# CornellHPC/HySortK

Hardware: AMD Instinct MI355X
Metric: k-mers counted/sec at K=31 (higher is better)
Workload: dtype u64

## Files before the change

hysortk_amd/csrc/hsk_api.hip:

```cpp
#include <hip/hip_runtime.h>
#include <dlfcn.h>
#include <algorithm>
#include <cstdarg>
#include <cstdio>
#include <cstdlib>
#include <cstring>
#include <future>
#include <map>
#include <string>
#include <thread>
#include <type_traits>
#include <vector>

#include "../../include/hsk.h"
#include "hsk_device.h"
#include "hsk_parse.h"
#include "hsk_expand.h"
#include "hsk_sort.h"
#include "hsk_scatter.h"
#include "hsk_count.h"
#include "hsk_finish.h"
#include "hsk_agg.h"
#include "hsk_combine.h"
#include "hsk_heavy.h"
#include "hsk_pairs.h"
#include "hsk_pairmerge.h"
#include "hsk_pairdiag.h"
#include "hsk_strand.h"
#include "hsk_estimate.h"
#include "hsk_synth.h"
#include "hsk_plan.h"
#include "hsk_tuning.h"
#include "hsk_comm.h"

using namespace hsk;

#include "hsk_pool.h"
#include "hsk_host_ctx.h"

extern "C" int hsk_abi_version(void) { return HSK_ABI_VERSION; }

extern "C" void *hsk_host_alloc(uint64_t bytes)
{
    void *p = nullptr;
    if (hipHostMalloc(&p, bytes ? bytes : 64, hipHostMallocDefault) != hipSuccess) { (void)hipGetLastError(); return nullptr; }
    return p;
}
extern "C" void hsk_host_free(void *p) { if (p) (void)hipHostFree(p); }

extern "C" int hsk_device_count(void)
{
    int n = 0;
    if (hipGetDeviceCount(&n) != hipSuccess) { (void)hipGetLastError(); return 0; }
    return n;
}

extern "C" const char *hsk_strerror(int s)
{
    switch (s) {
    case HSK_OK: return "ok";
    case HSK_ERR_INVALID_ARG: return "invalid argument";
    case HSK_ERR_NO_DEVICE: return "no usable HIP device (gfx950 required; there is no CPU fallback)";
    case HSK_ERR_HIP: return "HIP runtime error";
    case HSK_ERR_OOM: return "out of memory";
    case HSK_ERR_DISPATCH: return "Cannot dispatch tasks. May be too unbalanced.";
    case HSK_ERR_INTERNAL: return "internal device-side check failed";
    case HSK_ERR_COMM: return "RCCL communication error";
    case HSK_ERR_UNSUPPORTED: return "not supported";
    default: return "unknown status";
    }
}

extern "C" const char *hsk_last_error(const hsk_ctx *c) { return c ? c->err : ""; }

extern "C" void hsk_config_default(hsk_config *cfg)
{
    memset(cfg, 0, sizeof *cfg);
    cfg->kmer_size = 31; cfg->minimizer_size = 17; cfg->lower_freq = 15; cfg->upper_freq = 40;
    cfg->extension = 0; cfg->ntasks = 0; cfg->device = 0; cfg->plain_dispatcher = 0;
    cfg->dispatch_upper_coe = 1.5; cfg->dispatch_step = 0.05; cfg->radix_bits = 8; cfg->flags = 0; cfg->unbalanced_ratio = 2.3;
}

static int validate_cfg(const hsk_config *cfg)
{
    const int K = cfg->kmer_size, M = cfg->minimizer_size;
    if (!(2 < K && K < 96) || (K % 32) == 0) return 0;
    if (!(0 < M && M < K) || (M % 32) == 0) return 0;
    if (!(0 < cfg->lower_freq && cfg->lower_freq <= cfg->upper_freq && cfg->upper_freq <= 65535)) return 0;
    if (cfg->extension != 0 && cfg->extension != 1) return 0;
    if (cfg->ntasks < 0 || cfg->ntasks > HSK_MAX_TASKS) return 0;
    if (cfg->radix_bits != 0 && (cfg->radix_bits < MIN_RADIX_BITS || cfg->radix_bits > MAX_RADIX_BITS)) return 0;
    return 1;
}

#include <execinfo.h>
#include <signal.h>
#include <unistd.h>
static void backtrace_on_abort(int sig)
{
    void *frames[64];
    const int n = backtrace(frames, 64);
    backtrace_symbols_fd(frames, n, 2);
    signal(sig, SIG_DFL);
    raise(sig);
}

static size_t roll_back(hsk_ctx *c, unsigned long long mark, hsk_result *outs, int nouts)
{
    (void)hipStreamSynchronize(c->stream); (void)hipStreamSynchronize(c->comm_stream); (void)hipStreamSynchronize(c->d2h_stream);
    for (int r = 0; r < nouts; ++r) hsk_result_free(c, &outs[r]);
    const size_t n = c->pool.rollback(mark);
    if (c->d_err) (void)hipMemsetAsync(c->d_err, 0, 4, c->stream);
    return n;
}

struct ApiCall {
    hsk_ctx *c; const char *name; bool ok; unsigned long long mark; size_t live_open;
    ApiCall(hsk_ctx *c_, const char *name_) : c(c_), name(name_)
    {
        ok = hipSetDevice(c->cfg.device) == hipSuccess;
        if (!ok) { (void)hipGetLastError(); fail(c, HSK_ERR_HIP, "hipSetDevice(%d) failed", c->cfg.device); }
        c->call = CallState();
        mark = c->pool.mark(); live_open = c->pool.bytes_live;
    }
    template <typename F> int run(F &&impl, hsk_result *outs = nullptr, int nouts = 0) { return end(ok ? impl() : HSK_ERR_HIP, outs, nouts); }
    int end(int rc, hsk_result *outs = nullptr, int nouts = 0)
    {
        size_t rolled = rc != HSK_OK ? roll_back(c, mark, outs, nouts) : 0;
        if (c->pool.redzone) {
            (void)hipStreamSynchronize(c->stream); (void)hipStreamSynchronize(c->comm_stream); (void)hipStreamSynchronize(c->d2h_stream);
            char msg[320];
            if (c->pool.check(msg, sizeof msg) != 0) {
                if (rc == HSK_OK) rolled = roll_back(c, mark, outs, nouts);
                rc = fail(c, HSK_ERR_INTERNAL, "%s", msg);
            }
            c->pool.flush();
        }
        if (timing_enabled())
            fprintf(stderr, "[hsk] call %s: rc %d, pool live %zu -> %zu bytes, %zu blocks rolled back, cached %zu mapped %zu peak %zu bytes\n", name, rc, live_open,
                    c->pool.bytes_live, rolled, c->pool.bytes_cached, c->pool.bytes_mapped(), c->pool.peak);
        if (c->call.roff_check.valid()) (void)c->call.roff_check.get();
        c->call = CallState();
        return rc;
    }
};

template <typename F> static int with_nw(int nw, F &&f)
{
    switch (nw) {
    case 1: return f(std::integral_constant<int, 1>());
    case 2: return f(std::integral_constant<int, 2>());
    default: return f(std::integral_constant<int, 3>());
    }
}

extern "C" int hsk_init(const hsk_config *cfg, hsk_ctx **out)
{
    if (getenv("HSK_BACKTRACE") && atoi(getenv("HSK_BACKTRACE")) != 0) { signal(SIGABRT, backtrace_on_abort); signal(SIGSEGV, backtrace_on_abort); }
    if (!cfg || !out) return HSK_ERR_INVALID_ARG;
    *out = nullptr;
    if (!validate_cfg(cfg)) return HSK_ERR_INVALID_ARG;
    int ndev = 0;
    if (hipGetDeviceCount(&ndev) != hipSuccess || ndev <= 0) { (void)hipGetLastError(); return HSK_ERR_NO_DEVICE; }
    if (cfg->device < 0 || cfg->device >= ndev) return HSK_ERR_NO_DEVICE;
    hipDeviceProp_t prop;
    if (hipGetDeviceProperties(&prop, cfg->device) != hipSuccess) return HSK_ERR_NO_DEVICE;
    if (strncmp(prop.gcnArchName, "gfx950", 6) != 0) return HSK_ERR_NO_DEVICE;
    hsk_ctx *c = new hsk_ctx();
    c->cfg = *cfg;
    if (c->cfg.radix_bits == 0) c->cfg.radix_bits = 8;
    if (c->cfg.dispatch_upper_coe <= 0) c->cfg.dispatch_upper_coe = 1.5;
    if (c->cfg.dispatch_step <= 0) c->cfg.dispatch_step = 0.05;
    if (!(c->cfg.unbalanced_ratio > 0)) c->cfg.unbalanced_ratio = 2.3;
    c->nw = (cfg->kmer_size + 31) / 32;
    c->tune.parse(cfg->tuning);
// ... 914 lines not shown
```

hysortk_amd/csrc/hsk_host_finish.h:

```cpp
#pragma once

struct TaskOut { u64 n = 0, npay = 0; u64 *entries = nullptr; u64 *payoff = nullptr; u32 *pos = nullptr; int32_t *rid = nullptr; bool failed = false; u64 pay_base = 0; };

template <int NW>
static int count_task_device(hsk_ctx *c, const u64 *keys, const u64 *vals, u64 n, u64 payoff_add, u64 *d_histo, u32 histo_len, TaskOut &out)
{
    out = TaskOut();
    if (n == 0) return HSK_OK;
    const bool ext = vals != nullptr;
    const u64 ntiles = (n + CNT_TILE - 1) / CNT_TILE;
    u64 *d_tile_cnt, *d_total;
    DALLOC(c, d_tile_cnt, u64 *, ntiles * 8);
    DALLOC(c, d_total, u64 *, 256);
    CountArgs a; memset(&a, 0, sizeof a);
    a.keys = keys; a.n = n; a.lower = (u32)c->cfg.lower_freq; a.upper = (u32)c->cfg.upper_freq;
    a.tile_cnt = d_tile_cnt; a.histo = d_histo; a.histo_len = histo_len; a.payoff_add = payoff_add;
    hipLaunchKernelGGL((count_kernel<NW, false, false>), dim3((u32)ntiles), dim3(CNT_THREADS), 0, c->stream, a);
    hipLaunchKernelGGL(count_scan_kernel, dim3(1), dim3(CNT_THREADS), 0, c->stream, d_tile_cnt, ntiles, d_total);
    u64 *tot = &staging(c)->total;
    HIPCHK(c, hipMemcpyAsync(tot, d_total, 8, hipMemcpyDeviceToHost, c->stream));
    HIPCHK(c, hsk_sync(c, c->stream));
    out.n = tot[0]; out.npay = ext ? n : 0;
    if (ext) {
        DALLOC(c, out.pos, u32 *, n * 4);
// ... 41 lines not shown
static void host_release(hsk_ctx *c, ResultPriv *rp, void *p)
{
    for (size_t i = 0; i < rp->host_blocks.size(); ++i) if (rp->host_blocks[i] == p) { rp->host_blocks.erase(rp->host_blocks.begin() + i); break; }
    c->hpool.release(p);
}

static bool finish_enabled(const hsk_ctx *c) { return !(c->cfg.flags & HSK_FLAG_FULL_SORT); }
static bool agg_enabled(const hsk_ctx *c) { return !(c->cfg.flags & (HSK_FLAG_NO_AGGREGATION | HSK_FLAG_FULL_SORT)); }
static u32 auto_ntasks(hsk_ctx *c, u64 packed_bytes, int nranks)
{
    u64 est = packed_bytes * 4 * (u64)std::max(nranks, 1);
    u64 t = (est + (1ULL << 28) - 1) >> 28;
    t = std::max<u64>(t, (u64)std::max(nranks, 1));
    const u64 per = 8ULL * (u64)std::max(nranks, 1);
    if (packed_bytes * 4 >= (1ULL << 25)) t = std::max(t, per);
    if (t >= per) t = (t + per - 1) / per * per;
    return (u32)std::min<u64>(std::max<u64>(t, 1), HSK_MAX_TASKS);
}

template <int NW>
static int finish_batch_device(hsk_ctx *c, BatchTask *bt, int K, u64 max_task, u64 *d_histo, u32 histo_len, TaskOut *outs)
{
    static_assert(NW == 1, "fused finish handles one-word keys");
    const u32 L = (u32)c->cfg.lower_freq;
    const u32 cap_t = (u32)FN_NL / L + 1;
    u64 ntiles[XCD_BATCH], cnt_off[XCD_BATCH + 1]; cnt_off[0] = 0;
    for (int i = 0; i < XCD_BATCH; ++i) { ntiles[i] = (bt[i].n + FN_TILE - 1) / FN_TILE; cnt_off[i + 1] = cnt_off[i] + ntiles[i] + 1; }
    const size_t ctl_bytes = 64;
    char *d_ctl = (char *)c->pool.alloc(ctl_bytes + cnt_off[XCD_BATCH] * 8 + 64);
    if (!d_ctl) return fail(c, HSK_ERR_OOM, "finish control block");
    HIPCHK(c, hipMemsetAsync(d_ctl, 0, ctl_bytes, c->stream));
    u32 *d_flags = (u32 *)d_ctl; u64 *d_cnt = (u64 *)(d_ctl + ctl_bytes);
    u64 *scratch[XCD_BATCH] = {nullptr}; bool own_scratch[XCD_BATCH] = {false};
    for (int i = 0; i < XCD_BATCH; ++i) {
        if (bt[i].n == 0) continue;
        const u64 need = ntiles[i] * (u64)cap_t * 16;
        if (need <= max_task * 8) scratch[i] = other_side(bt[i]);
        else { scratch[i] = (u64 *)c->pool.alloc(need + 64); own_scratch[i] = true; if (!scratch[i]) return fail(c, HSK_ERR_OOM, "finish scratch of %llu bytes", (unsigned long long)need); }
        FinishArgs a; memset(&a, 0, sizeof a);
        a.keys = bt[i].out_k; a.n = bt[i].n; a.scratch = scratch[i]; a.cap_t = cap_t; a.tile_cnt = d_cnt + cnt_off[i]; a.flags = d_flags + i;
        a.lower = L; a.upper = (u32)c->cfg.upper_freq; a.hi_shift = HYBRID_SHIFT;
        hipLaunchKernelGGL(finish_kernel, dim3((u32)ntiles[i]), dim3(FN_THREADS), 0, c->stream, a);
        hipLaunchKernelGGL(count_scan_kernel, dim3(1), dim3(CNT_THREADS), 0, c->stream, d_cnt + cnt_off[i], ntiles[i], d_cnt + cnt_off[i] + ntiles[i]);
    }
    HIPCHK(c, hipGetLastError());
    struct { u32 flags[8]; u64 total[8]; } h; memset(&h, 0, sizeof h);
    HIPCHK(c, hipMemcpyAsync(h.flags, d_flags, sizeof h.flags, hipMemcpyDeviceToHost, c->stream));
    for (int i = 0; i < XCD_BATCH; ++i) if (bt[i].n) HIPCHK(c, hipMemcpyAsync(&h.total[i], d_cnt + cnt_off[i] + ntiles[i], 8, hipMemcpyDeviceToHost, c->stream));
    HIPCHK(c, hsk_sync(c, c->stream));
    static int occ = 0;
    if (!occ) { int nb = 0; occ = (hipOccupancyMaxActiveBlocksPerMultiprocessor(&nb, finish_compact_kernel, FN_THREADS, 0) == hipSuccess && nb > 0) ? nb : 4; }
    int rc = HSK_OK;
    for (int i = 0; i < XCD_BATCH && rc == HSK_OK; ++i) {
        outs[i] = TaskOut();
        if (bt[i].n == 0) continue;
        if (h.flags[i] && c->forbid_long_way) { outs[i].failed = true; continue; }
        if (h.flags[i]) {
            if (own_scratch[i]) { c->pool.release(scratch[i]); scratch[i] = nullptr; own_scratch[i] = false; }
            rc = long_way_task<NW>(c, bt[i], K, false, [&](u64 *sk, u64 *) { return count_task_device<NW>(c, sk, nullptr, bt[i].n, 0, d_histo, histo_len, outs[i]); });
            continue;
        }
        c->stats.fused_tasks++;
        outs[i].n = h.total[i];
        if (outs[i].n) {
            outs[i].entries = (u64 *)c->pool.alloc(outs[i].n * 16);
            if (!outs[i].entries) { rc = fail(c, HSK_ERR_OOM, "task output of %llu bytes", (unsigned long long)(outs[i].n * 16)); break; }
            const u32 grid = (u32)std::min<u64>((ntiles[i] + 3) / 4, (u64)occ * 256);
            hipLaunchKernelGGL(finish_compact_kernel, dim3(grid), dim3(FN_THREADS), 0, c->stream, scratch[i], cap_t, d_cnt + cnt_off[i], ntiles[i],
                               outs[i].entries, d_histo, histo_len);
        }
    }
    HIPCHK(c, hipGetLastError());
    HIPCHK(c, hsk_sync(c, c->stream));
    for (int i = 0; i < XCD_BATCH; ++i) if (own_scratch[i]) c->pool.release(scratch[i]);
    c->pool.release(d_ctl);
    return rc;
}

struct AggHostRead { u32 flags[AG_BATCH]; u32 maxd[AG_BATCH]; u32 ovf[2][AG_BATCH]; u32 large[2]; u64 total[AG_BATCH]; };
static_assert(sizeof(AggHostRead) <= sizeof PinnedTail().agg[0], "a slot of the pinned staging words holds one AggHostRead");
static_assert(sizeof(AggLarge) * AG_BATCH <= sizeof PinnedTail().agg_large[0], "... and a slot of agg_large the batch's AggLarge structs");

struct OvfLists {
    u32 *list[2] = {nullptr, nullptr};
    u32 *len[2] = {nullptr, nullptr};
    const u32 *h_len[2] = {nullptr, nullptr};
    u32 nbins = 0; int w = 0;
    u32 *appends(int i) const { return list[w] + (size_t)nbins * i; }
    u32 *appends_n(int i = 0) const { return len[w] + i; }
    const u32 *reads(int i) const { return list[w ^ 1] + (size_t)nbins * i; }
    const u32 *reads_n(int i) const { return len[w ^ 1] + i; }
    u32 appended(int i) const { return h_len[w][i]; }
    void swap() { w ^= 1; }
};
static bool first_table_up(hsk_ctx *c, int first_cap, int top, u64 ovf_bins, u64 all_bins)
{
    if (ovf_bins * 20 > all_bins) { c->agg_first_cap = std::min(first_cap + 1, top); c->agg_clean_batches = 0; return true; }
    return false;
}
static void first_table_down(hsk_ctx *c, int first_cap, u64 ovf_bins, const u32 *fullest)
{
    if (ovf_bins || first_cap <= AG_LOG2CAP_SMALL) return;
    if (fullest ? *fullest < (1u << (first_cap - 1)) * 3 / 4 : ++c->agg_clean_batches >= 4) { c->agg_first_cap = first_cap - 1; c->agg_clean_batches = 0; }
}
static bool ladder_hopeless(const hsk_ctx *c, int cap, u64 listed, u64 all_bins, bool &off)
{
    if (c->tune.agg_adapt == 0 || cap < AG_LOG2CAP_MEDIUM || listed * 2 <= all_bins) return false;
    return off = true;
}

struct AggPending {
    bool active = false;
    BatchTask bt[AG_BATCH];
    AggArgs a;
    u64 *d_bounds = nullptr, *d_cnt = nullptr, *d_off = nullptr; u32 *d_flags = nullptr;
    OvfLists ovf;
    char *d_large = nullptr;
    bool own_scratch[AG_BATCH] = {false};
    int first_cap = AG_LOG2CAP_SMALL;
    bool weighted = false;
    u32 nbins = 0, slot_shift = 0; int K = 0; u64 ntot = 0;
    hipEvent_t ev = nullptr;
    AggHostRead *h = nullptr;
};
template <int NW>
static int long_way_batch(hsk_ctx *c, const BatchTask *bt, const bool *redo, int K, const u64 *pay_before, u64 *d_histo, u32 histo_len, TaskOut *outs)
{
    BatchTask b2[XCD_BATCH];
    for (int i = 0; i < XCD_BATCH; ++i) {
        b2[i] = bt[i];
        if (!redo[i]) { b2[i].n = 0; continue; }
        if (bt[i].out_k != bt[i].kA) { std::swap(b2[i].kA, b2[i].kB); std::swap(b2[i].vA, b2[i].vB); }
        c->stats.redone_tasks++;
    }
    const auto counted = c->stats.redone_tasks;
    int rc = sort_batch_device<NW>(c, b2, K, false);
    c->stats.redone_tasks = counted;
    for (int i = 0; i < XCD_BATCH && rc == HSK_OK; ++i)
        if (redo[i]) rc = count_task_device<NW>(c, b2[i].out_k, b2[i].out_v, bt[i].n, pay_before ? pay_before[i] : 0, d_histo, histo_len, outs[i]);
    return rc;
}

constexpr int AG_LOG2CAP_HUGE = 13;
static_assert(Tuning().agg_maxrung == AG_LOG2CAP_HUGE, "the table's default of agg_maxrung (hsk_tuning.h) is the last rung");

template <typename F>
static void with_cap(int log2cap, F &&f)
{
    if (log2cap == AG_LOG2CAP_SMALL) f(std::integral_constant<int, AG_LOG2CAP_SMALL>{});
    else if (log2cap == AG_LOG2CAP_MEDIUM) f(std::integral_constant<int, AG_LOG2CAP_MEDIUM>{});
    else f(std::integral_constant<int, AG_LOG2CAP_LARGE>{});
}

template <int NW>
static int agg_launch_rung(hsk_ctx *c, AggPending &p, int log2cap, u32 grid_x, u64 records)
{
    const AggArgs &a = p.a; const dim3 grid(grid_x, AG_BATCH), block(AG_THREADS);
    profiled(c, 2, records, records * (NW * 8 + (p.weighted ? 8 : 0)), [&] {
        if constexpr (NW == 1) if (log2cap == AG_LOG2CAP_HUGE && !p.weighted) { hipLaunchKernelGGL(agg_big_kernel, grid, dim3(AGB_THREADS), 0, c->stream, a); return; }
        with_cap(log2cap, [&](auto cap) {
            constexpr int CAP = decltype(cap)::value;
            if constexpr (NW >= 2) {
                if constexpr (NW == 2) if (p.weighted) { hipLaunchKernelGGL((aggw_finish_kernel<CAP, NW, true>), grid, block, 0, c->stream, a); return; }
                hipLaunchKernelGGL((aggw_finish_kernel<CAP, NW>), grid, block, 0, c->stream, a);
            } else { if (p.weighted) hipLaunchKernelGGL((agg_finish_kernel<CAP, true>), grid, block, 0, c->stream, a); else hipLaunchKernelGGL((agg_finish_kernel<CAP>), grid, block, 0, c->stream, a); }
        });
    });
    HIPCHK(c, hipGetLastError());
    return HSK_OK;
}
static int agg_launch_scan(hsk_ctx *c, AggPending &p)
{
    hipLaunchKernelGGL(agg_scan_kernel, dim3(AG_BATCH), dim3(AG_THREADS), 0, c->stream, p.a);
    HIPCHK(c, hipGetLastError());
    HIPCHK(c, hipMemcpyAsync(p.h->flags, p.d_flags, offsetof(AggHostRead, total), hipMemcpyDeviceToHost, c->stream));
    HIPCHK(c, hipMemcpy2DAsync(p.h->total, 8, p.d_off + p.nbins, ((size_t)p.nbins + 8) * 8, 8, AG_BATCH, hipMemcpyDeviceToHost, c->stream));
    return HSK_OK;
}

template <int NW>
static int agg_large_setup(hsk_ctx *c, AggArgs &a, int slot, bool ext, char *&d_large)
{
    d_large = nullptr;
    u64 nmax = 0; for (int i = 0; i < AG_BATCH; ++i) if (a.t[i].active) nmax = std::max(nmax, a.t[i].n);
    if (c->tune.agg_large == 0 || nmax < AG_LARGE_BIN) return HSK_OK;
    const u32 nbins = a.nbins;
    const size_t tab8 = (size_t)AGL_TABLES * AGL_TAB * 8, tab4 = (size_t)AGL_TABLES * AGL_TAB * 4;
    size_t off[AG_BATCH][8], total = (sizeof(AggLarge) * AG_BATCH + 255) / 256 * 256;
    for (int i = 0; i < AG_BATCH; ++i) {
        const size_t sz[8] = {(size_t)nbins * 4, tab8, tab4 * (ext ? 3 : 1), 256, (size_t)(a.t[i].n / AGL_SLICE + AGL_TABLES + 1) * 8, 256, NW >= 2 ? tab8 : 0, NW == 3 ? tab8 : 0};
        for (int q = 0; q < 8; ++q) { off[i][q] = total; total += (sz[q] + 255) / 256 * 256; }
    }
    DALLOC(c, d_large, char *, total + 64);
    HIPCHK(c, hipMemsetAsync(d_large, 0, total, c->stream));
    AggLarge *h_lg = (AggLarge *)staging(c)->agg_large[slot];
    for (int i = 0; i < AG_BATCH; ++i) {
        HIPCHK(c, hipMemsetAsync(d_large + off[i][1], 0xFF, tab8, c->stream));
        if (NW == 2) HIPCHK(c, hipMemsetAsync(d_large + off[i][6], 0xFF, tab8, c->stream));
        AggLarge &g = h_lg[i];
        g.tkeys0 = NW >= 2 ? (unsigned long long *)(d_large + off[i][6]) : nullptr; g.tkeys1 = NW == 3 ? (unsigned long long *)(d_large + off[i][7]) : nullptr;
        g.bin_tab = (u32 *)(d_large + off[i][0]); g.tkeys = (unsigned long long *)(d_large + off[i][1]); g.tcnt = (u32 *)(d_large + off[i][2]);
        g.tbad = (u32 *)(d_large + off[i][3]); g.units = (unsigned long long *)(d_large + off[i][4]); g.ctl = (u32 *)(d_large + off[i][5]);
        a.t[i].lg = (const AggLarge *)d_large + i;
    }
    HIPCHK(c, hipMemcpyAsync(d_large, h_lg, sizeof(AggLarge) * AG_BATCH, hipMemcpyHostToDevice, c->stream));
    hipLaunchKernelGGL(agg_large_list_kernel, dim3(nbins / AG_THREADS + 1, AG_BATCH), dim3(AG_THREADS), 0, c->stream, a);
    hipLaunchKernelGGL(agg_large_slice_kernel<NW>, dim3(160, AG_BATCH), dim3(AG_THREADS), 0, c->stream, a);
    HIPCHK(c, hipGetLastError());
    return HSK_OK;
}

template <int NW>
static int agg_stage1(hsk_ctx *c, const BatchTask *bt, int K, int prefix_bits, int slot, AggPending &p, bool weighted = false)
{
    static_assert(NW <= 3, "the aggregating finish handles keys of one to three words");
    constexpr u32 EW = NW + 1;
    p = AggPending();
    const u32 L = (u32)c->cfg.lower_freq;
    p.weighted = weighted;
    p.slot_shift = (L >= 2 && !weighted) ? 1 : 0;
    p.nbins = 1u << prefix_bits; p.K = K;
    p.h = (AggHostRead *)staging(c)->agg[slot];
    memset(p.h, 0, sizeof *p.h);
    const u32 nbins = p.nbins;
    const size_t per = (size_t)nbins + 8;
    DALLOC(c, p.d_bounds, u64 *, per * 8 * AG_BATCH);
    DALLOC(c, p.d_cnt, u64 *, per * 8 * AG_BATCH);
    DALLOC(c, p.d_off, u64 *, per * 8 * AG_BATCH);
    DALLOC(c, p.d_flags, u32 *, 256);
    HIPCHK(c, hipMemsetAsync(p.d_flags, 0, 256, c->stream));
    OvfLists &ovf = p.ovf; ovf.nbins = nbins;
    for (int x = 0; x < 2; ++x) { DALLOC(c, ovf.list[x], u32 *, (size_t)nbins * 4 * AG_BATCH); ovf.len[x] = p.d_flags + (2 + x) * AG_BATCH; ovf.h_len[x] = p.h->ovf[x]; }
    AggArgs &a = p.a; memset(&a, 0, sizeof a);
    a.lower = L; a.upper = (u32)c->cfg.upper_freq; a.nbins = nbins; a.shift = 64 - prefix_bits; a.nw = NW;
    a.top_bits = (NW >= 2 && prefix_bits == 16) ? prefix_top_bits(K, NW) : 0;
    a.top_sig = NW >= 2 ? 2 * (K - 32 * (NW - 1)) : 64;
    u64 nmax = 0;
    for (int i = 0; i < AG_BATCH; ++i) {
        AggTask &t = a.t[i];
        p.bt[i] = bt[i];
        if (bt[i].n == 0) continue;
        t.keys = bt[i].out_k; t.vals = weighted ? bt[i].out_v : nullptr; t.n = bt[i].n; t.bounds = p.d_bounds + per * i; t.bin_cnt = p.d_cnt + per * i; t.bin_off = p.d_off + per * i; t.flags = p.d_flags + i;
        t.slot_shift = p.slot_shift; t.active = 1; p.ntot += bt[i].n; nmax = std::max(nmax, bt[i].n);
        t.ovf_list = ovf.appends(i); t.ovf_n = ovf.appends_n(i);
        if (p.slot_shift) t.scratch = other_side(bt[i]);
        else {
            t.scratch = (u64 *)c->pool.alloc(bt[i].n * EW * 8 + 64); p.own_scratch[i] = true;
            if (!t.scratch) return fail(c, HSK_ERR_OOM, "finish scratch of %llu bytes", (unsigned long long)(bt[i].n * EW * 8));
        }
    }
    hipLaunchKernelGGL(bin_bounds_kernel<AggArgs>, dim3(nbins / AG_THREADS + 1, AG_BATCH), dim3(AG_THREADS), 0, c->stream, a);
    if (!weighted) {
        a.lstat = p.d_flags + 4 * AG_BATCH;
        int rc = agg_large_setup<NW>(c, a, slot, false, p.d_large); if (rc) return rc;
    }
    p.first_cap = std::max(c->agg_first_cap, nmax / nbins >= 6144 ? AG_LOG2CAP_LARGE : AG_LOG2CAP_SMALL);
    if (weighted) {
        const u64 avg = nmax / nbins + 1;
        p.first_cap = avg * 2 <= 600 ? AG_LOG2CAP_SMALL : avg * 2 <= 1200 ? AG_LOG2CAP_MEDIUM : AG_LOG2CAP_LARGE;
    }
    int rc = agg_launch_rung<NW>(c, p, p.first_cap, nbins, p.ntot); if (rc) return rc;
    rc = agg_launch_scan(c, p); if (rc) return rc;
    p.ev = ev_get(c);
    HIPCHK(c, hipEventRecord(p.ev, c->stream));
    p.active = true;
    return HSK_OK;
}

template <int NW>
static int merge_sorted_pairs(hsk_ctx *c, const u64 *sk, const u64 *sv, u64 n, u64 *d_histo, u32 histo_len, TaskOut &out)
{
    out = TaskOut();
    if (n == 0) return HSK_OK;
    const u64 ntiles = (n + HV_THREADS - 1) / HV_THREADS;
    u64 *d_tile, *d_total;
    DALLOC(c, d_tile, u64 *, ntiles * 8 + 64); DALLOC(c, d_total, u64 *, 256);
    HeavyMergeArgs a; memset(&a, 0, sizeof a);
    a.keys = sk; a.cnts = sv; a.n = n; a.lower = (u64)c->cfg.lower_freq; a.upper = (u64)c->cfg.upper_freq; a.tile_cnt = d_tile; a.histo = d_histo; a.histo_len = histo_len;
    hipLaunchKernelGGL((heavy_merge_kernel<NW, false>), dim3((u32)ntiles), dim3(HV_THREADS), 0, c->stream, a);
    hipLaunchKernelGGL(count_scan_kernel, dim3(1), dim3(CNT_THREADS), 0, c->stream, d_tile, ntiles, d_total);
    u64 *tot = &staging(c)->total;
    HIPCHK(c, hipMemcpyAsync(tot, d_total, 8, hipMemcpyDeviceToHost, c->stream));
    HIPCHK(c, hsk_sync(c, c->stream));
    out.n = tot[0];
    if (out.n) {
        DALLOC(c, out.entries, u64 *, out.n * (NW + 1) * 8);
        a.entries = out.entries;
        hipLaunchKernelGGL((heavy_merge_kernel<NW, true>), dim3((u32)ntiles), dim3(HV_THREADS), 0, c->stream, a);
    }
    HIPCHK(c, hipGetLastError());
    c->pool.release(d_tile); c->pool.release(d_total);
    return HSK_OK;
}

template <int NW>
static int agg_stage2(hsk_ctx *c, AggPending &p, u64 *d_histo, u32 histo_len, TaskOut *outs, bool covered)
{
    constexpr u32 EW = NW + 1;
    for (int i = 0; i < AG_BATCH; ++i) outs[i] = TaskOut();
    if (!p.active) return HSK_OK;
    AggArgs &a = p.a; const BatchTask *bt = p.bt; const u32 nbins = p.nbins; OvfLists &ovf = p.ovf;
    bool &agg_off = NW == 1 ? c->agg_off : c->agg_off_wide;
    c->stats.host_syncs++; if (covered) c->stats.host_waits_covered++;
    HIPCHK(c, hipEventSynchronize(p.ev));
    ev_put(c, p.ev); p.ev = nullptr;
    AggHostRead &h = *p.h;
    bool done[AG_BATCH];
    int rc = HSK_OK, nact = 0;
    u64 ovf_bins = 0;
    for (int i = 0; i < AG_BATCH; ++i) { done[i] = bt[i].n == 0 || !h.flags[i]; if (bt[i].n) { ++nact; ovf_bins += ovf.appended(i); } }
    const u64 all_bins = (u64)nact * nbins;
    if (!c->forbid_long_way && !p.weighted && nact) {
        u32 maxd = 0; for (int i = 0; i < AG_BATCH; ++i) if (bt[i].n) maxd = std::max(maxd, h.maxd[i]);
        if (!first_table_up(c, p.first_cap, AG_LOG2CAP_LARGE, ovf_bins, all_bins)) first_table_down(c, p.first_cap, ovf_bins, NW == 1 ? &maxd : nullptr);
    }
    if (c->tune.agg_adapt == 2 && !c->forbid_long_way && !p.weighted) agg_off = true;
    if (ovf_bins) {
        AggArgs keep = a;
        int cap = p.first_cap;
        u32 n_cur[AG_BATCH]; for (int i = 0; i < AG_BATCH; ++i) n_cur[i] = bt[i].n ? ovf.appended(i) : 0;
        for (;;) {
            u32 longest = 0; u64 nb = 0; for (int i = 0; i < AG_BATCH; ++i) { longest = std::max(longest, n_cur[i]); nb += n_cur[i]; }
            if (!longest) break;
            const int max_rung = (int)c->tune.agg_maxrung;
            int next = (NW >= 2 || p.weighted) ? (cap < AG_LOG2CAP_LARGE ? cap + 1 : 0) : (cap < AG_LOG2CAP_HUGE ? cap + 1 : 0);
            if (next > max_rung) next = 0;
            if (!next) { for (int i = 0; i < AG_BATCH; ++i) if (n_cur[i]) done[i] = false; break; }
            if (!c->forbid_long_way && !p.weighted && ladder_hopeless(c, cap, nb, all_bins, agg_off)) {
                for (int i = 0; i < AG_BATCH; ++i) if (n_cur[i]) done[i] = false;
                break;
            }
            cap = next; ovf.swap();
            const bool last = (NW >= 2 || p.weighted) ? cap == AG_LOG2CAP_LARGE : cap == AG_LOG2CAP_HUGE;
            HIPCHK(c, hipMemsetAsync(ovf.appends_n(), 0, sizeof(u32) * AG_BATCH, c->stream));
            for (int i = 0; i < AG_BATCH; ++i) {
                AggTask &t = a.t[i];
                t.active = (keep.t[i].active && n_cur[i]) ? 1 : 0;
                if (t.active) c->stats.agg_retried_tasks++;
                t.bin_list = ovf.reads(i); t.bin_list_n = ovf.reads_n(i);
                t.ovf_list = last ? nullptr : ovf.appends(i); t.ovf_n = ovf.appends_n(i);
            }
            rc = agg_launch_rung<NW>(c, p, cap, longest, nb * (p.ntot / all_bins + 1)); if (rc) return rc;
            HIPCHK(c, hipMemcpyAsync(p.h->flags, p.d_flags, offsetof(AggHostRead, total), hipMemcpyDeviceToHost, c->stream));
            HIPCHK(c, hsk_sync(c, c->stream));
            if (last) { for (int i = 0; i < AG_BATCH; ++i) if (a.t[i].active && h.flags[i]) done[i] = false; break; }
            for (int i = 0; i < AG_BATCH; ++i) n_cur[i] = a.t[i].active ? ovf.appended(i) : 0;
        }
        a = keep;
        for (int i = 0; i < AG_BATCH; ++i) { a.t[i].bin_list = nullptr; a.t[i].bin_list_n = nullptr; }
        rc = agg_launch_scan(c, p); if (rc) return rc;
        HIPCHK(c, hsk_sync(c, c->stream));
    }
    u64 total[AG_BATCH];
    for (int i = 0; i < AG_BATCH; ++i) total[i] = h.total[i];
    c->stats.agg_large_bins += h.large[0]; c->stats.agg_large_slices += h.large[1];
    AggCompactArgs ca; memset(&ca, 0, sizeof ca);
    ca.slot_shift = p.slot_shift; ca.histo = d_histo; ca.histo_len = histo_len; ca.nbins = nbins; ca.ew = EW;
    bool any = false;
    for (int i = 0; i < AG_BATCH && rc == HSK_OK; ++i) {
        if (bt[i].n == 0 || !done[i]) continue;
        c->stats.fused_tasks++;
        outs[i].n = total[i];
        if (outs[i].n) {
            outs[i].entries = (u64 *)c->pool.alloc(outs[i].n * EW * 8);
            if (!outs[i].entries) { rc = fail(c, HSK_ERR_OOM, "task output of %llu bytes", (unsigned long long)(outs[i].n * EW * 8)); break; }
            ca.scratch[i] = a.t[i].scratch; ca.bounds[i] = a.t[i].bounds; ca.bin_off[i] = a.t[i].bin_off; ca.entries[i] = outs[i].entries;
            any = true;
        }
    }
    if (any && rc == HSK_OK) hipLaunchKernelGGL(agg_compact_kernel, dim3(256, AG_BATCH), dim3(AG_THREADS), 0, c->stream, ca);
    if (!c->forbid_long_way && !p.weighted && rc == HSK_OK) {
        bool redo[AG_BATCH]; int nredo = 0;
        for (int i = 0; i < AG_BATCH; ++i) { redo[i] = bt[i].n != 0 && !done[i]; nredo += redo[i]; }
        if (nredo >= 3) {
            for (int i = 0; i < AG_BATCH; ++i) if (redo[i] && p.own_scratch[i]) { c->pool.release(a.t[i].scratch); a.t[i].scratch = nullptr; p.own_scratch[i] = false; }
            rc = long_way_batch<NW>(c, bt, redo, p.K, nullptr, d_histo, histo_len, outs);
            for (int i = 0; i < AG_BATCH; ++i) if (redo[i]) done[i] = true;
        }
    }
    for (int i = 0; i < AG_BATCH && rc == HSK_OK; ++i) {
        if (bt[i].n == 0 || done[i]) continue;
        if (c->forbid_long_way) { outs[i].failed = true; continue; }
        if (p.own_scratch[i]) { c->pool.release(a.t[i].scratch); a.t[i].scratch = nullptr; p.own_scratch[i] = false; }
        rc = long_way_task<NW>(c, bt[i], p.K, p.weighted, [&](u64 *sk, u64 *sv) {
            return p.weighted ? merge_sorted_pairs<NW>(c, sk, sv, bt[i].n, d_histo, histo_len, outs[i])
                              : count_task_device<NW>(c, sk, nullptr, bt[i].n, 0, d_histo, histo_len, outs[i]); });
    }
    HIPCHK(c, hipGetLastError());
    for (int i = 0; i < AG_BATCH; ++i) if (p.own_scratch[i]) c->pool.release(a.t[i].scratch);
    c->pool.release(p.d_bounds); c->pool.release(p.d_cnt); c->pool.release(p.d_off); c->pool.release(p.d_flags); c->pool.release(ovf.list[0]); c->pool.release(ovf.list[1]); c->pool.release(p.d_large);
    p.active = false;
    return rc;
}

template <int NW>
static int agg_ext_finish_batch_device(hsk_ctx *c, BatchTask *bt, int K, const u64 *pay_before, u64 *d_histo, u32 histo_len, TaskOut *outs)
{
    static_assert(NW <= 3, "keys of one to three words");
    constexpr u32 EW = NW + 1;
    const u32 L = (u32)c->cfg.lower_freq;
    const u32 slot_shift = L >= 2 ? 1 : 0;
    const u32 nbins = AG_BINS;
    const size_t per = (size_t)nbins + 8;
    u64 *d_bounds, *d_cnt; u32 *d_flags;
    DALLOC(c, d_bounds, u64 *, per * 8 * AG_BATCH);
    DALLOC(c, d_cnt, u64 *, per * 8 * AG_BATCH);
    DALLOC(c, d_flags, u32 *, 256);
    HIPCHK(c, hipMemsetAsync(d_flags, 0, 256, c->stream));
    AggExtArgs a; memset(&a, 0, sizeof a);
    AggArgs sa; memset(&sa, 0, sizeof sa);
    a.lower = L; a.upper = (u32)c->cfg.upper_freq; a.nbins = nbins; a.shift = AG_SHIFT; a.nw = NW; a.top_bits = NW >= 2 ? prefix_top_bits(K, NW) : 0; a.top_sig = NW >= 2 ? 2 * (K - 32 * (NW - 1)) : 64;
    sa.nbins = nbins; sa.shift = AG_SHIFT; sa.nw = NW;
    bool own_scratch[AG_BATCH] = {false};
    u64 ntot = 0;
// ... 129 lines not shown
```

hysortk_amd/csrc/hsk_tuning.h:

```cpp
#pragma once
#include <stdlib.h>
#include <string.h>

namespace hsk {

#define HSK_TUNING_TABLE(X)                                                                                                              \
                                                                                              \
    X(parse_fast, 1)                                                                                   \
    X(parse_rec_cap, 0)              \
    X(scan_generic, 0)                                               \
    X(scan_place, 0)                                 \
    X(bin_cap_pct, 125)                  \
    X(bin_vmax, 0)                                                      \
    X(place_bytes, -1)                           \
    X(drop_certain, 1)                         \
                                                                             \
    X(zero_copy, 1)                                                      \
    X(uniform_len, 1)                                          \
    X(derive_offsets, 1)                                      \
    X(h2d_slabs, 16)                                   \
    X(ingest_pipeline, 1)                       \
                                                                              \
    X(plan_sample, 1)                                      \
    X(plan_min_input, 32LL << 20)          \
    X(xcd_batch, 1)                                                                    \
    X(force_no_xcd, 0)                                        \
    X(overlap, 1)                                        \
    X(lag, -1)                      \
    X(early_d2h, 1)                                                             \
    X(compact_d2h, 2)                                                           \
    X(widen_threads, 0)                           \
                                                     \
    X(expand_reserve, 1)               \
    X(unstable_first, 1)                                                        \
    X(wide_lookback, 0)                                                               \
    X(fused_scatter, 1)                                                         \
    X(fused_scatter_ext, 1)                                                                             \
    X(fused_scatter_wide, 1)                                                                         \
    X(xs2, 1)                                 \
    X(scatter_generic, 0)                                               \
                                                                                                 \
    X(agg_adapt, 1)                                               \
    X(agg_large, 1)                            \
    X(agg_maxrung, 13)                           \
                                                                     \
    X(combine, 1)                                                                                           \
    X(combine_dedup, 1)                                                 \
    X(combine_min_bytes, 64LL << 20)                                 \
    X(combine_bucket, 12288)                                                  \
    X(combine_ratio, 16)                                                   \
    X(combine_prefix, 0)                                   \
    X(pair_cap, 1)                                            \
    X(pair_cap_records, 0)                                            \
                                                                                                              \
    X(pool_redzone, 0)

struct Tuning {
#define X(name, dflt) long long name = dflt;
    HSK_TUNING_TABLE(X)
#undef X
#define X(name, dflt) bool name##_set = false;
    HSK_TUNING_TABLE(X)
#undef X

    void parse(const char *s)
    {
        while (s && *s) {
            const char *e = strchr(s, ',');
            const char *q = (const char *)memchr(s, '=', e ? (size_t)(e - s) : strlen(s));
            if (q && q > s) {
                const char *k = s; while (*k == ' ') ++k;
                set(k, (size_t)(q - k), atoll(q + 1));
            }
            s = e ? e + 1 : nullptr;
        }
    }

private:
    void set(const char *k, size_t n, long long value)
    {
#define X(name, dflt) if (n == sizeof(#name) - 1 && memcmp(k, #name, n) == 0) { if (!name##_set) { name = value; name##_set = true; } return; }
        HSK_TUNING_TABLE(X)
#undef X
    }
};

}
```

Measured before the change: 88.56 billion.

## Add a persistent pair-finish kernel for the first weighted aggregation rung

```diff
diff --git a/hysortk_amd/csrc/hsk_api.hip b/hysortk_amd/csrc/hsk_api.hip
--- a/hysortk_amd/csrc/hsk_api.hip
+++ b/hysortk_amd/csrc/hsk_api.hip
@@ -21,6 +21,7 @@
 #include "hsk_count.h"
 #include "hsk_finish.h"
 #include "hsk_agg.h"
+#include "hsk_pairfinish.h"
 #include "hsk_combine.h"
 #include "hsk_heavy.h"
 #include "hsk_pairs.h"
diff --git a/hysortk_amd/csrc/hsk_host_finish.h b/hysortk_amd/csrc/hsk_host_finish.h
--- a/hysortk_amd/csrc/hsk_host_finish.h
+++ b/hysortk_amd/csrc/hsk_host_finish.h
@@ -217,11 +217,23 @@
     else f(std::integral_constant<int, AG_LOG2CAP_LARGE>{});
 }
 
-template <int NW>
-static int agg_launch_rung(hsk_ctx *c, AggPending &p, int log2cap, u32 grid_x, u64 records)
+constexpr long long AGG_ADAPT_TABLES_ONLY = 3;
+template <int NW>
+static bool pair_finish_first(const hsk_ctx *c, bool weighted) { return NW == 1 && weighted && c->tune.agg_adapt != AGG_ADAPT_TABLES_ONLY; }
+static u32 pair_finish_grid(const AggArgs &a)
+{
+    static int occ = 0;
+    if (!occ) { int nb = 0; occ = (hipOccupancyMaxActiveBlocksPerMultiprocessor(&nb, pair_finish_kernel, AG_THREADS, 0) == hipSuccess && nb > 0) ? nb : 4; }
+    u32 nact = 0; for (int i = 0; i < AG_BATCH; ++i) nact += a.t[i].active ? 1u : 0u;
+    return std::min<u32>(a.nbins, std::max<u32>(1u, (u32)occ * 256u / std::max<u32>(nact, 1u)));
+}
+
+template <int NW>
+static int agg_launch_rung(hsk_ctx *c, AggPending &p, int log2cap, u32 grid_x, u64 records, bool first = false)
 {
     const AggArgs &a = p.a; const dim3 grid(grid_x, AG_BATCH), block(AG_THREADS);
     profiled(c, 2, records, records * (NW * 8 + (p.weighted ? 8 : 0)), [&] {
+        if constexpr (NW == 1) if (first && pair_finish_first<NW>(c, p.weighted)) { hipLaunchKernelGGL(pair_finish_kernel, dim3(pair_finish_grid(a), AG_BATCH), block, 0, c->stream, a); return; }
         if constexpr (NW == 1) if (log2cap == AG_LOG2CAP_HUGE && !p.weighted) { hipLaunchKernelGGL(agg_big_kernel, grid, dim3(AGB_THREADS), 0, c->stream, a); return; }
         with_cap(log2cap, [&](auto cap) {
             constexpr int CAP = decltype(cap)::value;
@@ -323,8 +335,10 @@
     if (weighted) {
         const u64 avg = nmax / nbins + 1;
         p.first_cap = avg * 2 <= 600 ? AG_LOG2CAP_SMALL : avg * 2 <= 1200 ? AG_LOG2CAP_MEDIUM : AG_LOG2CAP_LARGE;
-    }
-    int rc = agg_launch_rung<NW>(c, p, p.first_cap, nbins, p.ntot); if (rc) return rc;
+        static_assert(PF_CAP == 1u << AG_LOG2CAP_MEDIUM, "the first rung of the weighted finish counts as the medium one");
+        if (pair_finish_first<NW>(c, weighted)) p.first_cap = AG_LOG2CAP_MEDIUM;
+    }
+    int rc = agg_launch_rung<NW>(c, p, p.first_cap, nbins, p.ntot, true); if (rc) return rc;
     rc = agg_launch_scan(c, p); if (rc) return rc;
     p.ev = ev_get(c);
     HIPCHK(c, hipEventRecord(p.ev, c->stream));
diff --git a/hysortk_amd/csrc/hsk_pairfinish.h b/hysortk_amd/csrc/hsk_pairfinish.h
--- /dev/null
+++ b/hysortk_amd/csrc/hsk_pairfinish.h
@@ -0,0 +1,135 @@
+#pragma once
+#include "hsk_agg.h"
+#include "hsk_pairrank.h"
+
+namespace hsk {
+
+static_assert(PF_LANES == (u32)AG_THREADS, "hsk_pairrank.h counts the lanes of an aggregation workgroup");
+
+__global__ __launch_bounds__(AG_THREADS) void pair_finish_kernel(AggArgs a)
+{
+    __shared__ u64 s_key[PF_CAP];
+    __shared__ u32 s_cnt[PF_CAP];
+    __shared__ __attribute__((aligned(16))) u32 s_bkt[PF_NBKT];
+    __shared__ u32 s_start[PF_NBKT + 1];
+    __shared__ u32 s_bits[PF_WORDS];
+    const AggTask &t = a.t[blockIdx.y];
+    if (!t.active) return;
+    const int tid = threadIdx.x, lane = tid & (WAVE - 1), wave = tid >> 6;
+    const u32 b_lo = (u32)((u64)a.nbins * blockIdx.x / gridDim.x), b_hi = (u32)((u64)a.nbins * (blockIdx.x + 1) / gridDim.x);
+    if (b_lo >= b_hi) return;
+    const u64 *keys = t.keys, *vals = t.vals, *bounds = t.bounds;
+    u64 *bin_cnt = t.bin_cnt;
+    ulonglong2 *scratch = reinterpret_cast<ulonglong2 *>(t.scratch);
+    const u32 slot_shift = t.slot_shift, lower = a.lower, upper = a.upper;
+    const int shift = a.shift;
+
+    for (u32 i = tid; i < PF_NBKT; i += AG_THREADS) s_bkt[i] = 0;
+    if (tid < (int)PF_WORDS) s_bits[tid] = 0;
+
+    u32 vz = 0;
+    asm volatile("" : "+v"(vz));
+    auto uniform64 = [](u64 v) -> u64 {
+        return ((u64)(u32)__builtin_amdgcn_readfirstlane((int)(u32)(v >> 32)) << 32) | (u32)__builtin_amdgcn_readfirstlane((int)(u32)v);
+    };
+    auto load_bin = [&](u64 s, u32 n, u64 (&k)[PF_PER], u32 (&c)[PF_PER]) {
+#pragma unroll
+        for (u32 u = 0; u < PF_PER; ++u) {
+            k[u] = 0; c[u] = 0;
+            if (u * PF_LANES < n) {
+                const u32 i = u * PF_LANES + (u32)tid;
+                if (i < n) { k[u] = keys[s + i]; c[u] = (u32)vals[s + i]; }
+            }
+        }
+    };
+    auto bin_n = [](u64 s, u64 e) -> u32 { return e - s > (u64)PF_CAP ? PF_CAP + 1u : (u32)(e - s); };
+
+    u64 s = uniform64(bounds[b_lo + vz]), e = uniform64(bounds[b_lo + 1 + vz]);
+    u64 e_next = b_lo + 1 < b_hi ? bounds[b_lo + 2 + vz] : 0;
+    u64 k[PF_PER]; u32 c[PF_PER];
+    {
+        const u32 n0 = bin_n(s, e);
+        load_bin(s, n0 <= PF_CAP ? n0 : 0u, k, c);
+    }
+    lds_barrier();
+
+    for (u32 b = b_lo; b < b_hi; ++b) {
+        const u32 n = bin_n(s, e);
+        const bool more = b + 1 < b_hi;
+        const u64 s2 = e, e2 = more ? uniform64(e_next) : e;
+        const u32 n2 = bin_n(s2, e2);
+        u64 nk[PF_PER]; u32 nc[PF_PER];
+        load_bin(s2, n2 <= PF_CAP ? n2 : 0u, nk, nc);
+        u64 e_nn = b + 2 < b_hi ? bounds[b + 3 + vz] : 0;
+
+        if (n == 0) {
+            if (tid == 0) bin_cnt[b] = 0;
+        } else if (n > PF_CAP) {
+            if (tid == 0) { agg_bin_overflow(t, a.nbins, b); atomicMax(t.flags + AG_BATCH, PF_CAP); }
+        } else {
+            u32 ar[PF_PER];
+#pragma unroll
+            for (u32 u = 0; u < PF_PER; ++u) {
+                ar[u] = 0;
+                if (u * PF_LANES < n && u * PF_LANES + (u32)tid < n) ar[u] = atomicAdd(&s_bkt[pf_bucket(k[u], shift)], 1u);
+            }
+            lds_barrier();
+            {
+                const uint4 v0 = reinterpret_cast<const uint4 *>(s_bkt)[lane * 2], v1 = reinterpret_cast<const uint4 *>(s_bkt)[lane * 2 + 1];
+                const u32 v[8] = {v0.x, v0.y, v0.z, v0.w, v1.x, v1.y, v1.z, v1.w};
+                u32 sum = 0;
+#pragma unroll
+                for (int x = 0; x < 8; ++x) sum += v[x];
+                u32 ex = wave_incl_scan_dpp(sum) - sum;
+                if ((lane >> 4) == wave) {
+#pragma unroll
+                    for (int x = 0; x < 8; ++x) { s_start[lane * 8 + x] = ex; ex += v[x]; }
+                    if (tid == AG_THREADS - 1) s_start[PF_NBKT] = ex;
+                }
+            }
+            lds_barrier();
+#pragma unroll
+            for (u32 u = 0; u < PF_PER; ++u)
+                if (u * PF_LANES < n && u * PF_LANES + (u32)tid < n) {
+                    const u32 at = s_start[pf_bucket(k[u], shift)] + ar[u];
+                    s_key[at] = k[u]; s_cnt[at] = c[u];
+                }
+            for (u32 i = tid; i < PF_NBKT; i += AG_THREADS) s_bkt[i] = 0;
+            lds_barrier();
+            u32 keptm = 0;
+#pragma unroll
+            for (u32 u = 0; u < PF_PER; ++u) {
+                if (u * PF_LANES < n && u * PF_LANES + (u32)tid < n) {
+                    const u32 bk = pf_bucket(k[u], shift), b0 = s_start[bk], b1 = s_start[bk + 1u];
+                    PfRank r = {0, 0, 0};
+                    for (u32 q = b0; q < b1; ++q) pf_see(r, k[u], ar[u], s_key[q], q - b0, s_cnt[q]);
+                    ar[u] = pf_rank(b0, r); c[u] = r.sum;
+                    if (pf_keep(r, lower, upper)) { keptm |= 1u << u; atomicOr(&s_bits[pf_word(ar[u])], pf_bit(ar[u])); }
+                }
+            }
+            lds_barrier();
+            const u32 word = s_bits[lane];
+            const u32 pc = (u32)__builtin_popcount(word);
+            const u32 incl = wave_incl_scan_dpp(pc);
+            const u32 D = (u32)__builtin_amdgcn_readlane((int)incl, WAVE - 1);
+#pragma unroll
+            for (u32 u = 0; u < PF_PER; ++u) {
+                if (u * PF_LANES < n) {
+                    const u32 w = pf_word(ar[u]);
+                    const u32 ww = (u32)__shfl((int)word, (int)w, WAVE), before = (u32)__shfl((int)(incl - pc), (int)w, WAVE);
+                    if (keptm & (1u << u)) { const u32 o = pf_slot(before, ww, ar[u]); s_key[o] = k[u]; s_cnt[o] = c[u]; }
+                }
+            }
+            lds_barrier();
+            ulonglong2 *dst = scratch + (s >> slot_shift);
+            for (u32 i = tid; i < D; i += AG_THREADS) dst[i] = make_ulonglong2(s_key[i], (u64)s_cnt[i]);
+            if (tid == 0) bin_cnt[b] = D;
+            if (tid < (int)PF_WORDS) s_bits[tid] = 0;
+        }
+#pragma unroll
+        for (u32 u = 0; u < PF_PER; ++u) { k[u] = nk[u]; c[u] = nc[u]; }
+        s = s2; e = e2; e_next = e_nn;
+    }
+}
+
+}
diff --git a/hysortk_amd/csrc/hsk_pairrank.h b/hysortk_amd/csrc/hsk_pairrank.h
--- /dev/null
+++ b/hysortk_amd/csrc/hsk_pairrank.h
@@ -0,0 +1,42 @@
+#pragma once
+#include <stdint.h>
+
+#if defined(__HIPCC__)
+#define HSK_PAIRRANK_FN __host__ __device__ __forceinline__
+#else
+#define HSK_PAIRRANK_FN inline
+#endif
+
+namespace hsk {
+
+typedef uint64_t u64;
+typedef uint32_t u32;
+
+constexpr u32 PF_LANES = 256;
+constexpr u32 PF_PER = 8;
+constexpr u32 PF_CAP = PF_LANES * PF_PER;
+constexpr int PF_LOG2BKT = 9;
+constexpr u32 PF_NBKT = 1u << PF_LOG2BKT;
+constexpr u32 PF_WORDS = PF_CAP / 32;
+static_assert(PF_WORDS == 64, "a wave scans the mask's words, one per lane");
+static_assert(PF_NBKT == 64 * 8, "a wave scans the buckets, eight per lane");
+
+HSK_PAIRRANK_FN u32 pf_bucket(u64 key, int shift) { return (u32)(key >> (shift - PF_LOG2BKT)) & (PF_NBKT - 1u); }
+
+struct PfRank { u32 less, eq_before, sum; };
+HSK_PAIRRANK_FN void pf_see(PfRank &r, u64 mine, u32 my_arrival, u64 other, u32 other_arrival, u32 other_cnt)
+{
+    const bool eq = other == mine;
+    r.less += other < mine ? 1u : 0u;
+    r.eq_before += (eq && other_arrival < my_arrival) ? 1u : 0u;
+    r.sum += eq ? other_cnt : 0u;
+}
+HSK_PAIRRANK_FN u32 pf_rank(u32 b0, const PfRank &r) { return b0 + r.less + r.eq_before; }
+HSK_PAIRRANK_FN bool pf_head(const PfRank &r) { return r.eq_before == 0; }
+HSK_PAIRRANK_FN bool pf_keep(const PfRank &r, u32 lower, u32 upper) { return pf_head(r) && r.sum >= lower && r.sum <= upper; }
+
+HSK_PAIRRANK_FN u32 pf_word(u32 rank) { return rank >> 5; }
+HSK_PAIRRANK_FN u32 pf_bit(u32 rank) { return 1u << (rank & 31u); }
+HSK_PAIRRANK_FN u32 pf_slot(u32 words_before, u32 word, u32 rank) { return words_before + (u32)__builtin_popcount(word & (pf_bit(rank) - 1u)); }
+
+}
diff --git a/hysortk_amd/csrc/hsk_tuning.h b/hysortk_amd/csrc/hsk_tuning.h
--- a/hysortk_amd/csrc/hsk_tuning.h
+++ b/hysortk_amd/csrc/hsk_tuning.h
@@ -40,7 +40,7 @@
     X(xs2, 1)                                 \
     X(scatter_generic, 0)                                               \
                                                                                                  \
-    X(agg_adapt, 1)                                               \
+    X(agg_adapt, 1)                 \
     X(agg_large, 1)                            \
     X(agg_maxrung, 13)                           \
                                                                      \
```

New measurement: 91.07 billion, median of 6. 2.8% higher.
